# traupach/xarray_parcel

Measured on AMD Instinct MI355X. Metric: column-profiles/sec for surface_based_cape_cin, higher is better.
Workload: dtype f64

## Files before the change

xarray_parcel_amd/csrc/xp_cape_tu.hip:

```cpp
#include <hip/hip_runtime.h>

#include <cstdlib>

#include "xp_kernels.hpp"

#if !defined(XP_TU_T) || !defined(XP_TU_MODE)
#error "compile with -DXP_TU_T=<float|double> -DXP_TU_MODE=<0|1|2>"
#endif

namespace xp {
namespace {

int cape_block() {
    static int b = [] { const char *e = getenv("XP_CAPE_BLOCK"); int v = e ? atoi(e) : XP_CAPE_THREADS; return (v == 64 || v == 128 || v == 256 || v == XP_CAPE_THREADS) ? v : XP_CAPE_THREADS; }();
    return b;
}

template <typename T, int PM, int MODE, bool PERSIST> void launch_p(const CapeArgs &a, bool profile, hipStream_t s) {
    const int b = cape_block();
    unsigned nblk = (unsigned)((a.ncol + b - 1) / b);
    if (PERSIST) {
        static const int n_cu = [] { int d = 0; hipDeviceProp_t pr; return (hipGetDevice(&d) == hipSuccess && hipGetDeviceProperties(&pr, d) == hipSuccess) ? pr.multiProcessorCount : 256; }();
        unsigned cap = (unsigned)(n_cu * (b >= 1024 ? 1 : 1024 / b));
        if (nblk > cap) nblk = cap;
    }
    dim3 gr(nblk), bl(b);
    if (a.hum) {
        if (profile) hipLaunchKernelGGL((k_cape_cin<T, PM, true, MODE, true, false, false, PERSIST>), gr, bl, 0, s, a);
        else hipLaunchKernelGGL((k_cape_cin<T, PM, false, MODE, true, false, false, PERSIST>), gr, bl, 0, s, a);
        return;
    }
    if (profile) {
        if constexpr (MODE == 2) {
            const bool cc_only = !a.s.lfc_t && !a.s.el_t && !a.s.lfc_idx && !a.s.el_idx && !a.s.status;
            if (a.prof.nlev_out == 0 && a.prof.li && a.vtc && a.pos_neg && a.log_interp && cc_only) {
                hipLaunchKernelGGL((k_cape_cin<T, PM, true, MODE, false, true, true, PERSIST>), gr, bl, 0, s, a);
                return;
            }
        }
        hipLaunchKernelGGL((k_cape_cin<T, PM, true, MODE, false, false, false, PERSIST>), gr, bl, 0, s, a);
        return;
    }
    const bool lean = !a.s.lfc_t && !a.s.el_t && !a.s.lfc_idx && !a.s.el_idx && !a.s.status;
    const bool dflt = a.vtc && a.pos_neg && a.log_interp;
    if (dflt && lean) { hipLaunchKernelGGL((k_cape_cin<T, PM, false, MODE, false, true, true, PERSIST>), gr, bl, 0, s, a); return; }
    if constexpr (MODE != 2) {
        if (dflt) { hipLaunchKernelGGL((k_cape_cin<T, PM, false, MODE, false, true, false, PERSIST>), gr, bl, 0, s, a); return; }
    }
    hipLaunchKernelGGL((k_cape_cin<T, PM, false, MODE, false, false, false, PERSIST>), gr, bl, 0, s, a);
}
template <typename T, int PM, int MODE> void launch_t(const CapeArgs &a, bool profile, hipStream_t s) {
    if constexpr (MODE == 2) {
        if (a.persist) { launch_p<T, PM, MODE, true>(a, profile, s); return; }
    }
    launch_p<T, PM, MODE, false>(a, profile, s);
}

}

template <> void launch_cape_mode<XP_TU_T, XP_TU_MODE>(const CapeArgs &a, int pm, bool profile, hipStream_t s) {
    switch (pm) {
        case PM_SURFACE: launch_t<XP_TU_T, PM_SURFACE, XP_TU_MODE>(a, profile, s); break;
        case PM_MU: launch_t<XP_TU_T, PM_MU, XP_TU_MODE>(a, profile, s); break;
        case PM_ML: launch_t<XP_TU_T, PM_ML, XP_TU_MODE>(a, profile, s); break;
        default: launch_t<XP_TU_T, PM_EXPLICIT, XP_TU_MODE>(a, profile, s); break;
    }
}

}
```

xarray_parcel_amd/csrc/xp_kernels.hpp:

```cpp
#pragma once
#include "xp_level_reader.hpp"
#include "xp_profile_out.hpp"

namespace xp {

struct CapeArgs {
    View p, t, td;
    int64_t nlev, ncol;
    const void *ex_p, *ex_t, *ex_td;
    double depth;
    int vtc, log_interp, pos_neg, post_zero, table_mode;
    int hum;
    int off32;
    Tables tb;
    const double *es_tab;
    const double *fam_tab;
    int32_t *flags;
    int persist;
    int only_flagged;
    ScalarsOut s;
    ProfileOut prof;
};

enum { PM_SURFACE = 0, PM_MU = 1, PM_ML = 2, PM_EXPLICIT = 3 };


template <bool HUM> XP_DEV double as_dewpoint(const double *es, double p, double t, double m) {
    return HUM ? dewpoint_from_q_tab(es, p, t, m) : m;
}

template <typename T, bool HUM> XP_DEV Parcel select_mu_exact(const CapeArgs &a, int64_t c, const double *es, const double depth) {
    Parcel r; r.p = r.t = r.td = qnan(); r.first = a.nlev; r.idx = -1; r.prepend = false;
    double bottom = qnan(), bound = qnan(), dmin = qnan(), best = qnan();
    LookAhead<T> next(a.p, a.t, a.td, c, 0);
    for (int64_t k = 0; k < a.nlev; ++k) {
        double p, t, td;
        next.take(k + 1, a.nlev, p, t, td);
        td = as_dewpoint<HUM>(es, p, t, td);
        if (isnan_(p)) continue;
        if (isnan_(bottom)) { bottom = p; bound = bottom - depth; }
        double d = fabs(p - bound);
        bool below = p < bound;
        if (below && !(d < dmin)) break;
        if (!(d >= dmin)) dmin = d;
        double e = ln_theta_e(es, p, t, td);
        if (!isnan_(e) && !(e <= best)) { best = e; r.p = p; r.t = t; r.td = td; r.first = k; r.idx = (int)k; }
        if (below) break;
    }
    return r;
}
XP_DEV float ln_theta_e_f32(float p, float t, float td) {
    float e = 6.112f * __builtin_amdgcn_exp2f((17.67f - 4302.645f * __builtin_amdgcn_rcpf(td - 29.65f)) * 1.4426950408889634f);
    float r = 0.6219569100577033f * e * __builtin_amdgcn_rcpf(p - e);
    float l2t = __builtin_amdgcn_logf(t), l2td = __builtin_amdgcn_logf(td);
    float tl = 56.0f + __builtin_amdgcn_rcpf(__builtin_amdgcn_rcpf(td - 56.0f) + (l2t - l2td) * (0.6931471805599453f / 800.0f));
    float l2tl = __builtin_amdgcn_logf(tl);
    return 0.6931471805599453f * (l2t + (2.0f / 7.0f) * (9.965784284662087f - __builtin_amdgcn_logf(p - e)) + 0.28f * r * (l2t - l2tl)) +
// ... 85 lines not shown
    if (!closed) {
        double th_t = (pb == top) ? thb : qnan(), w_t = (pb == top) ? wb : qnan();
        layer_mean_step(s_th, pp, thp, top, th_t);
        layer_mean_step(s_w, pp, wp, top, w_t);
    }
    double dlay = fabs(top - bottom);
    double th_m = (1.0 / dlay) * s_th, w_m = (1.0 / dlay) * s_w;
    r.p = p_start;
    r.t = th_m * fpow(p_start / 1000.0, KAPPA);
    r.td = dewpoint_of_e(vapor_pressure(p_start, w_m));
    return r;
}

template <typename T, bool HUM> XP_DEV Parcel choose_parcel(const CapeArgs &a, int pmode, int64_t c, const double *es, const double depth) {
    Parcel pc;
    if (pmode == PM_SURFACE) {
        pc.p = ld<T>(a.p, 0, c); pc.t = ld<T>(a.t, 0, c); pc.td = as_dewpoint<HUM>(es, pc.p, pc.t, ld<T>(a.td, 0, c));
        pc.first = 0; pc.idx = 0; pc.prepend = false;
    } else if (pmode == PM_EXPLICIT) {
        pc.p = ld1<T>(a.ex_p, c); pc.t = ld1<T>(a.ex_t, c); pc.td = ld1<T>(a.ex_td, c);
        pc.first = 0; pc.idx = -1; pc.prepend = false;
    } else if (pmode == PM_MU) {
        pc = select_mu<T, HUM>(a, c, es, depth);
    } else {
        pc = select_ml<T, HUM>(a, c, es, depth);
    }
    return pc;
}

template <typename T, int PMODE, bool PROFILE, int MODE, bool HUM, bool DEF, bool LEAN, bool PERSIST>
__global__ __launch_bounds__(XP_CAPE_THREADS, (XP_CAPE_THREADS >= 1024 ? 4 : MODE == 2 ? 3 : PROFILE ? 4 : (PMODE == PM_SURFACE ? (HUM ? 3 : 1) : 4))) void k_cape_cin(CapeArgs a) {
    constexpr bool TABLE = (MODE == 1), FAMILY = (MODE == 2);
    constexpr bool LAZY = FAMILY && PROFILE && LEAN;
    struct Lds { double es[LDS_TAB]; double fam[FAMILY ? FAM_SIZE : 1]; double slot[SLOT_FIELDS * SLOT_STRIDE]; int next; };
    struct LdsRef { double *es, *fam, *slot; int *next; } lds;
    if constexpr (FAMILY && PROFILE) {
        __shared__ double l_es[LDS_TAB];
        __shared__ double l_fam[FAM_SIZE];
        __shared__ double l_slot[SLOT_FIELDS * SLOT_STRIDE];
        __shared__ int l_next;
        lds.es = l_es; lds.fam = l_fam; lds.slot = l_slot; lds.next = &l_next;
    } else {
        __shared__ Lds l;
        lds.es = l.es; lds.fam = l.fam; lds.slot = l.slot; lds.next = &l.next;
    }
    double *const s_es = lds.es;
    double *const s_fam = lds.fam;
    if (FAMILY) for (int i = threadIdx.x; i < FAM_SIZE; i += blockDim.x) s_fam[i] = a.fam_tab[i];
    int &s_next = *lds.next;
    if (PERSIST && threadIdx.x == 0) s_next = (int)(blockDim.x >> 6);
    int64_t c0 = (int64_t)blockIdx.x * blockDim.x + threadIdx.x;
    if (a.only_flagged) {
        int need = (c0 < a.ncol) ? a.flags[c0] : 0;
        if (!__syncthreads_or(need)) return;
        stage_es_table(a.es_tab, s_es);
        if (!need) return;
    } else {
        stage_es_table(a.es_tab, s_es);
        if (!PERSIST && c0 >= a.ncol) return;
    }
    const double *es = s_es;
    double *const s_slot = lds.slot;

    auto column = [&](const int64_t c) __attribute__((always_inline)) {
    const Parcel pc = choose_parcel<T, HUM>(a, PMODE, c, es, a.depth);

    const bool vtc = DEF || (a.vtc != 0), pos_neg = DEF || (a.pos_neg != 0), log_interp = DEF || (a.log_interp != 0);
    const bool need_w = vtc || PROFILE;
    const Lcl l = lcl(pc.p, pc.t, pc.td);
    int status = l.not_converged ? ST_LCL_NOT_CONVERGED : 0;
    const ScalarsOut &s = a.s;

    if (isnan_(l.p)) {
        if (PROFILE) ProfileSink<T, LAZY>::blank(a.prof, c);
        store_blank_column(s, c, pc, l, status);
        if (FAMILY) a.flags[c] = 0;
        return;
    }

    store_parcel_and_lcl(s, c, pc, l);
    const double vf_parcel = need_w ? virt_factor_tab(es, pc.t, pc.td, pc.p, false) : 1.0;
    const double x_lcl = log(l.p);
    const double x0 = (pc.p == l.p) ? x_lcl : log_tab<true>(es, pc.p);

    Scan sc; sc.init(l.p, x_lcl, pos_neg, s_slot + threadIdx.x);
    sc.slot[SL_LCL_T * SLOT_STRIDE] = vtc ? l.tv : l.t;
    Moist m;
    Family fam;
    if (FAMILY) fam.start(s_fam, es, l.p, x_lcl, l.t, l.tv);
    else m.start(es, l.p, x_lcl, l.t, TABLE, a.tb);
    double fam_off = l.tv - l.t;
    double fam_offp = fam_off;

    ProfileSink<T, LAZY> sink;
    constexpr bool TRACK = LEAN && PMODE == PM_ML;
    int last_k = -1, cur_k = -1;
    auto emit = [&](auto above, double P, double X, double tp, double tvp, double te, double tve, double tde, bool is_lcl) __attribute__((always_inline)) {
        if (PROFILE) sink.node(a.prof, c, es, sc, P, X, tp, tvp, te, tve, tde);
        if (TRACK) {
            if (!isnan_(P)) { last_k = (is_lcl || cur_k < 0) ? -1 : cur_k; if (is_lcl || cur_k < 0) sc.slot[SL_MIN_P * SLOT_STRIDE] = P; }
        }
        sc.template node<LEAN, decltype(above)::value>(P, X, vtc ? tvp : tp, vtc ? tve : te, is_lcl);
    };

    bool lcl_done = false;
    double *const br = sc.slot;
    clear_bracket(br);
    auto moist_node = [&](double P, double X, double T_, double m_, bool Q) __attribute__((always_inline)) {
        constexpr bool TRIO = FAMILY && LEAN && !PROFILE && !HUM && (PMODE == PM_SURFACE || PMODE == PM_EXPLICIT);
        bool f_top = false, f_any_top = false;
        const double fz = TRIO ? fam.locate(X, f_top, f_any_top) : 0.0;
        double tf = TRIO ? 0.0 : FAMILY ? fam.at(X) : m.at(P, X, a.tb, true);
        constexpr bool PARCEL_ES = TABLE;
        constexpr bool FAM_T = FAMILY && PROFILE;
        unsigned dist = table_dist(T_);
        if (!Q) dist = umax_(dist, table_dist(m_));
        if (PARCEL_ES && need_w) dist = umax_(dist, table_dist(tf));
        const bool in_range = all_in_table(dist) && (!FAM_T || LAZY || in_table(tf, 8.0));
// ... 112 lines not shown
            double Pn, Tn, Mn;
            rd.take(rem > 1, Pn, Tn, Mn);
            if (ku >= resume) {
                if (TRACK) cur_k = ku - 1;
                moist_node(sP, log_tab<true>(es, sP), sT, Q ? sM : as_dewpoint<HUM>(es, sP, sT, sM), Q);
                sP = Pn; sT = Tn; sM = Mn;
            }
        }
    } else {
        plain_walk(k);
    }
    if (TRACK) {
        if (last_k >= 0) sc.slot[SL_MIN_P * SLOT_STRIDE] = ld<T>(a.p, last_k, c);
    } else if (LEAN) {
        double pm = l.p;
        bool found = false;
        if constexpr (!SEARCH) {
            const double q = rd.peek_p();
            if (!isnan_(q)) { pm = (q < pm) ? q : pm; found = true; }
        }
        const auto late_in = late_kernargs<CapeArgs>();
        const View top_p = {late_in->p.data, late_in->p.ls, late_in->p.cs};
        for (int kk = nlev - 1; kk >= (int)pc.first; --kk) {
            if (__ballot(!found) == 0ull) break;
            const double q = ld<T>(top_p, kk, c);
            if (!found && !isnan_(q)) { pm = (q < pm) ? q : pm; found = true; }
        }
        sc.slot[SL_MIN_P * SLOT_STRIDE] = pm;
    }
    if (PROFILE) sink.finish(a.prof, c);

    const auto late = late_kernargs<CapeArgs>();
    Scan::Result r = sc.finish(late->post_zero != 0);
    if (FAMILY) late->flags[c] = fam.bad ? 1 : 0;
    store_scan_result(late->s, c, r, status | r.status);
    };

    if (PERSIST) persistent_tiles(a.ncol, s_next, column);
    else column(c0);
}

template <typename T, int PMODE> __global__ __launch_bounds__(256) void k_select_parcel(CapeArgs a) {
    __shared__ double s_es[LDS_TAB];
    const double *es = stage_es_table(a.es_tab, s_es);
    int64_t c = (int64_t)blockIdx.x * blockDim.x + threadIdx.x;
    if (c >= a.ncol) return;
    Parcel pc = choose_parcel<T, false>(a, PMODE, c, es, a.depth);
    st(a.s.par_p, a.s.f64, c, pc.p); st(a.s.par_t, a.s.f64, c, pc.t); st(a.s.par_td, a.s.f64, c, pc.td);
    sti(a.s.parcel_idx, c, pc.idx);
}

template <typename T> __global__ __launch_bounds__(256)
void k_mixed_layer(View pv, View vv, int64_t nlev, int64_t ncol, double depth_in, void *out, int f64) {
    int64_t c = (int64_t)blockIdx.x * blockDim.x + threadIdx.x;
    if (c >= ncol) return;
    double bottom = qnan(), top = qnan(), s = 0.0, pp = qnan(), vp = qnan(), pb = qnan(), vb = qnan();
    bool closed = false;
    for (int64_t k = 0; k < nlev; ++k) {
        double p = ld<T>(pv, k, c), v = ld<T>(vv, k, c);
        if (isnan_(bottom) && !isnan_(p)) { bottom = p; top = bottom - depth_in; }
        if (!isnan_(p) && p < top) {
            double cb = flog(pb), ca = flog(p), va = v;
            if (pb == top) { ca = cb; va = vb; }
            layer_mean_step(s, pp, vp, top, interp_rule(vb, va, flog(top), cb, ca));
            closed = true;
            break;
        }
        if (k > 0) layer_mean_step(s, pp, vp, p, v);
        pp = p; vp = v;
        if (!isnan_(p)) { pb = p; vb = v; }
    }
    if (!closed) layer_mean_step(s, pp, vp, top, (pb == top) ? vb : qnan());
// ... 294 lines not shown
```

xarray_parcel_amd/csrc/xp_lcl_node.hpp:

```cpp
#pragma once
#include "xp_device.hpp"

namespace xp {

struct View { const void *data; int64_t ls, cs; };
struct OutView { void *data; int64_t ls, cs; };

template <typename T> XP_DEV double ld(const View &v, int64_t k, int64_t c) {
    return (double)((const T *)v.data)[k * v.ls + c * v.cs];
}
template <typename T> XP_DEV T ldr(const View &v, int64_t k, int64_t c) { return ((const T *)v.data)[k * v.ls + c * v.cs]; }
template <typename T> XP_DEV double ld1(const void *p, int64_t c) { return (double)((const T *)p)[c]; }
XP_DEV void st(void *p, int f64, int64_t i, double v) {
    if (p == nullptr) return;
    if (f64) ((double *)p)[i] = v; else ((float *)p)[i] = (float)v;
}
XP_DEV void sti(int32_t *p, int64_t i, int v) { if (p) p[i] = v; }

struct ScalarsOut {
    void *cape, *cin, *lcl_p, *lcl_t, *lcl_tv, *lfc_p, *lfc_t, *el_p, *el_t;
    int32_t *lfc_idx, *el_idx, *status, *parcel_idx;
    void *par_p, *par_t, *par_td;
    int f64;
};
// ... 5 lines not shown
    sti(s.parcel_idx, c, pc.idx);
    st(s.par_p, s.f64, c, pc.p); st(s.par_t, s.f64, c, pc.t); st(s.par_td, s.f64, c, pc.td);
}
template <typename S> XP_DEV void store_blank_column(const S &s, int64_t c, const Parcel &pc, const Lcl &l, int status) {
    st(s.cape, s.f64, c, 0.0); st(s.cin, s.f64, c, 0.0);
    st(s.lfc_p, s.f64, c, qnan()); st(s.lfc_t, s.f64, c, qnan()); st(s.el_p, s.f64, c, qnan()); st(s.el_t, s.f64, c, qnan());
    sti(s.lfc_idx, c, -1); sti(s.el_idx, c, -1); sti(s.status, c, status);
    store_parcel_and_lcl(s, c, pc, l);
}
template <typename S> XP_DEV void store_scan_result(const S &s, int64_t c, const Scan::Result &r, int status) {
    const int f64 = s.f64;
    st(s.cape, f64, c, r.cape); st(s.cin, f64, c, r.cin);
    st(s.lfc_p, f64, c, r.lfc_p); st(s.lfc_t, f64, c, r.lfc_t);
    st(s.el_p, f64, c, r.el_p); st(s.el_t, f64, c, r.el_t);
    sti(s.lfc_idx, c, r.lfc_idx); sti(s.el_idx, c, r.el_idx); sti(s.status, c, status);
}

template <typename Args> XP_DEV const Args __attribute__((address_space(4))) *late_kernargs() {
    typedef const Args __attribute__((address_space(4))) *KernargPtr;
    KernargPtr late = (KernargPtr)__builtin_amdgcn_kernarg_segment_ptr();
    asm volatile("" : "+s"(late) : : "memory");
    return late;
}

template <typename F> XP_DEV void persistent_tiles(int64_t ncol, int &s_next, const F &column) {
    const int64_t ntiles = (ncol + 63) >> 6;
    const int t0 = (int)(ntiles * blockIdx.x / gridDim.x), t1 = (int)(ntiles * (blockIdx.x + 1) / gridDim.x);
    int tile = t0 + (int)(threadIdx.x >> 6);
    while (tile < t1) {
        const int64_t c = ((int64_t)tile << 6) + (threadIdx.x & 63);
        if (c < ncol) column(c);
        if ((threadIdx.x & 63) == 0) tile = t0 + atomicAdd(&s_next, 1);
        tile = __builtin_amdgcn_readfirstlane(tile);
    }
}

XP_DEV double interp_rule(double xb, double xa, double at, double cb, double ca) {
    double res = xb + (xa - xb) * fdiv(at - cb, ca - cb);
    return (xb == xa) ? xb : res;
}

XP_DEV void snap_to_lcl(const double *es, double lp, double x_lcl, double &P, double &X) {
    if (fabs(P - lp) <= LCL_SNAP * lp) P = lp;
    X = log_tab<true>(es, P);
    X = (P == lp) ? x_lcl : X;
}

XP_DEV void clear_bracket(double *br) {
    br[SL_BR_P * SLOT_STRIDE] = qnan(); br[SL_BR_X * SLOT_STRIDE] = qnan(); br[SL_BR_T * SLOT_STRIDE] = qnan(); br[SL_BR_TD * SLOT_STRIDE] = qnan();
}
XP_DEV void store_bracket(double *br, double P, double X, double T_, double Td_) {
    br[SL_BR_P * SLOT_STRIDE] = P; br[SL_BR_X * SLOT_STRIDE] = X; br[SL_BR_T * SLOT_STRIDE] = T_; br[SL_BR_TD * SLOT_STRIDE] = Td_;
}
XP_DEV void lcl_environment(const double *br, bool log_interp, double lp, double x_lcl, double pa, double xa, double ta, double tda,
                            double &te, double &tde) {
    const double at = log_interp ? x_lcl : lp;
    const double pb = br[SL_BR_P * SLOT_STRIDE], xb = br[SL_BR_X * SLOT_STRIDE], tb_ = br[SL_BR_T * SLOT_STRIDE], tdb = br[SL_BR_TD * SLOT_STRIDE];
    lds_wait_all();
    double cb = log_interp ? xb : pb, ca = log_interp ? xa : pa;
    if (pb == lp) { ca = cb; ta = tb_; tda = tdb; }
    te = interp_rule(tb_, ta, at, cb, ca); tde = interp_rule(tdb, tda, at, cb, ca);
}

template <bool PAIR = false> XP_DEV double virt_env_ranged(const double *es, double T_, double Td_, double P) {
    if (__builtin_amdgcn_ballot_w64(!all_in_table(umax_(table_dist(T_), table_dist(Td_)))) == 0ull) return virt_env_tab<PAIR>(es, T_, Td_, P, true);
    double tq = T_;
// ... 64 lines not shown
```

xarray_parcel_amd/csrc/xparcel.hip:

```cpp
#include <hip/hip_runtime.h>

#include <cstdarg>
#include <cstdio>
#include <cmath>
#include <cstring>
#include <cstdlib>
#include <algorithm>
#include <mutex>
#include <vector>

#include "../../include/xparcel.h"
#include "xp_kernels.hpp"
#include "xp_cape_f32.hpp"
#include "xp_multi.hpp"
#include "xp_bundle.hpp"
#include "xp_dcape.hpp"
#include "xp_kinematics.hpp"
#include "xp_effective.hpp"
#include "xp_cape_layers.hpp"
#include "xp_wind_layers.hpp"
#include "xp_thermo_layers.hpp"
#include "xp_sounding.hpp"
#include "xp_isentropic.hpp"
#include "xp_hydrostatic.hpp"
// ... 311 lines not shown
int stage_scalars(Stager &st, xp_scalars_out *s, int64_t ncol, xp::ScalarsOut *o) {
    memset(o, 0, sizeof(*o));
    if (!s) { o->f64 = 1; return 0; }
    if (s->dtype != XP_F32 && s->dtype != XP_F64) return fail(XP_E_ARG, "scalars: bad dtype");
    o->f64 = s->dtype == XP_F64;
    size_t fb = (size_t)ncol * esize(s->dtype), ib = (size_t)ncol * 4;
    int rc = 0;
#define F_(dst, src) if (!rc) rc = st.out(s->src, fb, s->mem, &o->dst)
#define I_(dst, src) if (!rc) rc = st.out(s->src, ib, s->mem, &o->dst)
    F_(cape, cape); F_(cin, cin); F_(lcl_p, lcl_pressure); F_(lcl_t, lcl_temperature); F_(lcl_tv, lcl_virtual_temperature);
    F_(lfc_p, lfc_pressure); F_(lfc_t, lfc_temperature); F_(el_p, el_pressure); F_(el_t, el_temperature);
    I_(lfc_idx, lfc_index); I_(el_idx, el_index); I_(status, status); I_(parcel_idx, parcel_index);
    F_(par_p, parcel_pressure); F_(par_t, parcel_temperature); F_(par_td, parcel_dewpoint);
#undef F_
#undef I_
    return rc;
}

struct TableSet { xp::Tables tb; const double *es, *fam; };
int snapshot_tables(bool table_mode, TableSet *t) {
    std::lock_guard<std::mutex> lk(g.mu);
    if (table_mode && !g.tables) return fail(XP_E_NO_TABLES, "Call load_moist_adiabat_lookups first.");
    *t = {g.tb, g.es_tab, g.fam_tab};
    return 0;
}

bool persist(int mode, int64_t ncol) {
    static const long long env = [] { const char *e = getenv("XP_PERSIST_MIN_COLS"); return e ? atoll(e) : -1ll; }();
    const bool searching = mode < 0 || mode == XP_PARCEL_MOST_UNSTABLE || mode == XP_PARCEL_MIXED_LAYER;
    const long long min_cols = env >= 0 ? env : searching ? (1ll << 19) : (3ll << 18);
    return (long long)ncol >= min_cols && ncol < (1ll << 36);
}

template <typename T, int PM> void launch_cape(const xp::CapeArgs &a, bool profile, hipStream_t s) {
    if (a.ncol == 0) return;
    if (a.table_mode) xp::launch_cape_mode<T, 1>(a, PM, profile, s);
    else if (a.flags) {
        xp::launch_cape_mode<T, 2>(a, PM, profile, s);
        xp::CapeArgs b = a;
        b.only_flagged = 1;
        xp::launch_cape_mode<T, 0>(b, PM, profile, s);
    } else xp::launch_cape_mode<T, 0>(a, PM, profile, s);
}
template <typename T> void launch_cape_pm(const xp::CapeArgs &a, int pm, bool profile, hipStream_t s) {
    switch (pm) {
        case XP_PARCEL_SURFACE: launch_cape<T, xp::PM_SURFACE>(a, profile, s); break;
        case XP_PARCEL_MOST_UNSTABLE: launch_cape<T, xp::PM_MU>(a, profile, s); break;
        case XP_PARCEL_MIXED_LAYER: launch_cape<T, xp::PM_ML>(a, profile, s); break;
        default: launch_cape<T, xp::PM_EXPLICIT>(a, profile, s); break;
    }
}

xp_opts default_opts() {
    xp_opts o;
    memset(&o, 0, sizeof(o));
    o.virtual_temperature_correction = 1; o.lcl_interp = XP_LCL_INTERP_LOG; o.pos_cape_neg_cin = 1; o.compute = XP_F64;
    return o;
}
int check_opts(const xp_opts &o, bool f32_ok = false) {
    if (o.lcl_interp != XP_LCL_INTERP_LINEAR && o.lcl_interp != XP_LCL_INTERP_LOG)
        return fail(XP_E_INTERP, "interpolator must be linear or log");
    if (o.moist_mode != XP_MOIST_EXACT && o.moist_mode != XP_MOIST_TABLE && o.moist_mode != XP_MOIST_FAMILY)
        return fail(XP_E_ARG, "bad moist_mode");
    if (o.compute != XP_F64 && !(f32_ok && o.compute == XP_F32))
        return fail(XP_E_ARG, o.compute == XP_F32 ? "xp_opts.compute: XP_F32 arithmetic is implemented by xp_cape_cin only" : "xp_opts.compute: XP_F32 or XP_F64");
    if (o.humidity != XP_HUM_DEWPOINT && o.humidity != XP_HUM_SPECIFIC) return fail(XP_E_ARG, "bad xp_opts.humidity");
    return 0;
}
int check_parcel(const xp_parcel *parcel) {
    if (!parcel) return fail(XP_E_ARG, "parcel: null");
    if (parcel->mode < XP_PARCEL_SURFACE || parcel->mode > XP_PARCEL_EXPLICIT) return fail(XP_E_ARG, "parcel: bad mode");
    if (parcel->mode == XP_PARCEL_EXPLICIT && (!parcel->pressure || !parcel->temperature || !parcel->dewpoint))
        return fail(XP_E_ARG, "explicit parcel: null arrays");
    return 0;
}
int check_cape(const xp_view *p, const xp_view *t, const xp_view *td, int np, const xp_parcel *parcels, const xp_opts &o, bool f32_ok = false) {
    if (int rc = check_views({{p, "pressure"}, {t, "temperature"}, {td, "dewpoint"}})) return rc;
    for (int i = 0; i < np; ++i)
        if (int rc = check_parcel(parcels + i)) return rc;
    return check_opts(o, f32_ok);
}

// ... 38 lines not shown
                const xp_opts &o, xp::CapeArgs *a, bool f32_ok = false) {
    int rc;
    if ((rc = check_cape(p, t, td, 1, parcel, o, f32_ok)) || (rc = stage_cape(st, p, t, td, o, a)) || (rc = set_parcel(st, *parcel, p, a)))
        return rc;
    return 0;
}
int stage_cape_out(Stager &st, int dtype, xp_scalars_out *scalars, xp_profile_out *profile, xp::CapeArgs *a) {
    int rc;
    if ((rc = stage_scalars(st, scalars, a->ncol, &a->s)) || !profile) return rc;
    if (profile->dtype != XP_F32 && profile->dtype != XP_F64) return fail(XP_E_ARG, "profile: bad dtype");
    if (profile->nlev_out < a->nlev + 1) return fail(XP_E_ARG, "profile: nlev_out must be >= nlev + 1");
    if (profile->mem == XP_MEM_HOST && !(profile->col_stride == 1 && profile->lev_stride == a->ncol))
        return fail(XP_E_ARG, "profile: host arrays must be dense (nlev_out, ncol)");
    void *src[6] = {profile->pressure, profile->temperature, profile->virtual_temperature,
                    profile->environment_temperature, profile->environment_virtual_temperature,
                    profile->environment_dewpoint};
    size_t b = (size_t)profile->nlev_out * (size_t)a->ncol * esize(profile->dtype);
    int rows = 0;
    for (int v = 0; v < 6; ++v) {
        if ((rc = st.out(src[v], b, profile->mem, &a->prof.v[v]))) return rc;
        rows += a->prof.v[v] != nullptr;
    }
    a->prof.nlev_out = rows ? profile->nlev_out : 0;
    a->prof.ls = profile->lev_stride; a->prof.cs = profile->col_stride;
    a->prof.f64 = profile->dtype == XP_F64;
    a->prof.native6 = rows == 6 && profile->dtype == dtype;
    if (profile->lifted_index) {
        if (!(profile->lifted_index_pressure > 0.0)) return fail(XP_E_ARG, "profile: lifted_index_pressure must be positive");
        if ((rc = st.out(profile->lifted_index, (size_t)a->ncol * esize(profile->dtype), profile->mem, &a->prof.li))) return rc;
        a->prof.li_x = log(profile->lifted_index_pressure);
    }
    return 0;
}
int family_flags(Stager &st, const xp_opts &o, int64_t ncol, int32_t **flags) {
    *flags = nullptr;
    if (o.moist_mode != XP_MOIST_FAMILY || ncol == 0) return 0;
    return st.alloc(sizeof(int32_t) * (size_t)ncol, flags);
}
void cape_pass(const Stager &st, xp::CapeArgs a, int dtype, int mode, bool profile, int32_t *flags) {
    a.flags = flags;
    a.persist = flags && persist(mode, a.ncol);
    by_dtype(dtype, [&](auto z) { launch_cape_pm<decltype(z)>(a, mode, profile, st.s); });
}

int check_compute32(const xp_view *p, const xp_parcel *parcel, const xp_opts &o, const xp_scalars_out *s, const xp_profile_out *profile) {
    if (p->dtype != XP_F32) return fail(XP_E_ARG, "xp_opts.compute = XP_F32: the views must be XP_F32");
    if (parcel->mode != XP_PARCEL_SURFACE) return fail(XP_E_ARG, "xp_opts.compute = XP_F32: parcel->mode must be XP_PARCEL_SURFACE");
    if (o.moist_mode != XP_MOIST_FAMILY) return fail(XP_E_ARG, "xp_opts.compute = XP_F32: moist_mode must be XP_MOIST_FAMILY");
    if (o.humidity != XP_HUM_DEWPOINT) return fail(XP_E_ARG, "xp_opts.compute = XP_F32: humidity must be XP_HUM_DEWPOINT");
    if (!o.virtual_temperature_correction || o.lcl_interp != XP_LCL_INTERP_LOG || !o.pos_cape_neg_cin || o.post_zero_cin)
        return fail(XP_E_ARG, "xp_opts.compute = XP_F32: virtual_temperature_correction, lcl_interp, pos_cape_neg_cin and post_zero_cin must be at their defaults");
    if (profile) return fail(XP_E_ARG, "xp_opts.compute = XP_F32: profile must be NULL");
    if (s && (s->lfc_temperature || s->el_temperature || s->lfc_index || s->el_index || s->status))
        return fail(XP_E_ARG, "xp_opts.compute = XP_F32: scalars->lfc_temperature, el_temperature, lfc_index, el_index and status must be NULL");
    return 0;
}
void cape_pass32(const Stager &st, xp::CapeArgs a, int32_t *flags) {
    if (a.ncol == 0) return;
    a.flags = flags;
    a.persist = persist(XP_PARCEL_SURFACE, a.ncol);
    xp::launch_cape_f32(a, st.s);
    a.only_flagged = 1; a.persist = 0;
    xp::launch_cape_mode<float, 0>(a, xp::PM_SURFACE, false, st.s);
}

template <typename T, int NV> void launch_interp_levels(int nt, const Stager &st, const xp::View &cv, const xp::InterpMany &m, int64_t nlev, int64_t ncol, int lg) {
    switch (nt) {
        case 1: launch(xp::k_interp_levels<T, NV, 1>, ncol, st, cv, m, nlev, ncol, lg); break;
        case 2: launch(xp::k_interp_levels<T, NV, 2>, ncol, st, cv, m, nlev, ncol, lg); break;
        case 3: launch(xp::k_interp_levels<T, NV, 3>, ncol, st, cv, m, nlev, ncol, lg); break;
        default: launch(xp::k_interp_levels<T, NV, 4>, ncol, st, cv, m, nlev, ncol, lg); break;
    }
}
template <typename T> void launch_interp_levels_v(int nv, int nt, const Stager &st, const xp::View &cv, const xp::InterpMany &m, int64_t nlev, int64_t ncol, int lg) {
    switch (nv) {
// ... 127 lines not shown
    g.tb.p_max = t->p_max; g.tb.p_step = t->p_step; g.tb.t_min = t->t_min; g.tb.t_step = t->t_step;
    g.tables = true;
    return XP_OK;
}
int xp_tables_loaded(void) { return g.tables ? 1 : 0; }

int xp_family_table(double *out, int64_t *n_lnp, int64_t *n_label) {
    DevGuard dg_;
    int rc = ensure_init();
    if (rc) return rc;
    if (n_lnp) *n_lnp = xp::FAM_COEFS / xp::FAM_NPS;
    if (n_label) *n_label = xp::FAM_NPS;
    if (out) memcpy(out, g.fam_host.data(), sizeof(double) * xp::FAM_COEFS);
    return XP_OK;
}
int xp_set_family_table(const double *tab, int64_t n_lnp, int64_t n_label) {
    DevGuard dg_;
    int rc = ensure_init();
    if (rc) return rc;
    if (!tab || n_lnp != xp::FAM_COEFS / xp::FAM_NPS || n_label != xp::FAM_NPS) return fail(XP_E_ARG, "xp_set_family_table: wrong shape");
    std::lock_guard<std::mutex> lk(g.mu);
    HIP_TRY(hipDeviceSynchronize());
    memcpy(g.fam_host.data(), tab, sizeof(double) * xp::FAM_COEFS);
    HIP_TRY(hipMemcpy(g.fam_tab, family_device_layout(g.fam_host).data(), sizeof(double) * g.fam_host.size(), hipMemcpyHostToDevice));
    return XP_OK;
}

int xp_cape_cin(const xp_view *p, const xp_view *t, const xp_view *td, const xp_parcel *parcel, const xp_opts *o,
                xp_scalars_out *scalars, xp_profile_out *profile, void *stream) {
    Entry st(stream);
    if (st.rc) return st.rc;
    const xp_opts oo = o ? *o : default_opts();
    xp::CapeArgs a;
    int32_t *flags;
    int rc;
    const bool f32 = oo.compute == XP_F32;
    if (f32 && ((rc = check_cape(p, t, td, 1, parcel, oo, true)) || (rc = check_compute32(p, parcel, oo, scalars, profile)))) return rc;
    if ((rc = fill_common(st, p, t, td, parcel, oo, &a, true)) || (rc = stage_cape_out(st, p->dtype, scalars, profile, &a)) ||
        (rc = family_flags(st, oo, a.ncol, &flags))) return rc;
    if (f32) cape_pass32(st, a, flags);
    else cape_pass(st, a, p->dtype, parcel->mode, profile != nullptr, flags);
    return st.finish();
}

int xp_cape_cin_multi(const xp_view *p, const xp_view *t, const xp_view *td, int32_t np, const xp_parcel *parcels,
                      const xp_opts *o, xp_scalars_out *scalars, xp_profile_out *profiles, void *stream) {
    Entry st(stream);
    if (st.rc) return st.rc;
    if (np < 1 || np > xp::MULTI_MAX) return fail(XP_E_ARG, "xp_cape_cin_multi: 1...%d parcels", xp::MULTI_MAX);
    if (!parcels || !scalars) return fail(XP_E_ARG, "xp_cape_cin_multi: null parcels / scalars");
    const xp_opts oo = o ? *o : default_opts();
    xp::CapeArgs a, pa[xp::MULTI_MAX];
    int rc;
    if ((rc = check_cape(p, t, td, np, parcels, oo)) || (rc = stage_cape(st, p, t, td, oo, &a))) return rc;
    for (int i = 0; i < np; ++i) {
        pa[i] = a;
        if ((rc = set_parcel(st, parcels[i], p, &pa[i])) ||
            (rc = stage_cape_out(st, p->dtype, &scalars[i], profiles ? &profiles[i] : nullptr, &pa[i]))) return rc;
    }
    const int64_t ncol = a.ncol;
    if (!multi_fused_ok(np, parcels, oo, profiles)) {
        int32_t *flags;
        if ((rc = family_flags(st, oo, ncol, &flags))) return rc;
        for (int i = 0; i < np; ++i) cape_pass(st, pa[i], p->dtype, parcels[i].mode, profiles != nullptr, flags);
        return st.finish();
    }
    xp::MultiArgs m;
    memset(&m, 0, sizeof(m));
    m.base = a;
    m.np = np;
    for (int i = 0; i < np; ++i) {
        m.mode[i] = parcels[i].mode;
        m.depth[i] = parcels[i].depth;
        m.s[i] = pa[i].s;
    }
    if (ncol == 0) return st.finish();
    int32_t *flags;
    if ((rc = st.alloc(sizeof(int32_t) * (size_t)ncol * (size_t)np, &flags))) return rc;
    for (int i = 0; i < np; ++i) m.flags[i] = flags + (size_t)i * (size_t)ncol;
    m.base.persist = persist(-1, ncol);
    by_dtype(p->dtype, [&](auto z) {
        using T = decltype(z);
        xp::launch_cape_multi<T, 2>(m, st.s);
        for (int i = 0; i < np; ++i) {
            xp::CapeArgs b = pa[i];
            b.flags = m.flags[i]; b.only_flagged = 1;
            xp::launch_cape_mode<T, 0>(b, m.mode[i], false, st.s);
        }
    });
    return st.finish();
}

int xp_conv_properties(const xp_conv_in *in, const xp_opts *o, int32_t ignore_nans, xp_conv_out *out, void *stream) {
    Entry st(stream);
    if (st.rc) return st.rc;
    if (!in || !out) return fail(XP_E_ARG, "xp_conv_properties: null argument");
// ... 20 lines not shown
        if ((rc = st.in(src[i]->data, rows_bytes(src[i], src[i]->nlev), mem, &d))) return rc;
        dv[i].data = d; dv[i].mem = XP_MEM_DEVICE;
    }
    const void *sfu, *sfv;
    if ((rc = st.in(in->surface_wind_u, cb, mem, &sfu)) || (rc = st.in(in->surface_wind_v, cb, mem, &sfv))) return rc;
    void *td, *tmp;
    int32_t *valid;
    enum { T850, T700, T500, TD850, Z700, Z500, HIU, HIV, MUP, MUTD, NTMP };
    if ((rc = st.alloc((size_t)nlev * cb, &td)) || (rc = st.alloc((size_t)NTMP * cb, &tmp)) || (rc = st.alloc((size_t)ncol * 4, &valid))) return rc;
    auto tp = [&](int i) { return (void *)((char *)tmp + (size_t)i * cb); };
    void *o_[21];
    void *const want[21] = {out->mu_cape, out->mu_cin, out->mu_mixing_ratio, out->mu_lifted_index, out->mu_dci,
                            out->mixed_100_cape, out->mixed_100_cin, out->mixed_100_lifted_index, out->mixed_100_dci,
                            out->mixed_50_cape, out->mixed_50_cin, out->mixed_50_lifted_index, out->mixed_50_dci,
                            out->lapse_rate_700_500, out->temp_500, out->freezing_level, out->melting_level,
                            out->shear_u, out->shear_v, out->shear_magnitude, (void *)out->positive_shear};
    for (int i = 0; i < 21; ++i) {
        const size_t b = i == 20 ? (size_t)ncol * 4 : cb;
        if ((rc = want[i] ? st.out(want[i], b, mem, &o_[i]) : st.alloc(b, &o_[i]))) return rc;
    }
    enum { O_MU_CAPE, O_MU_CIN, O_MU_W, O_MU_LI, O_MU_DCI, O_M1_CAPE, O_M1_CIN, O_M1_LI, O_M1_DCI, O_M5_CAPE, O_M5_CIN, O_M5_LI, O_M5_DCI,
           O_LAPSE, O_T500, O_FRZ, O_MLT, O_SHU, O_SHV, O_SHM, O_POS };
    xp::ConvColumnsArgs ca;
    memset(&ca, 0, sizeof(ca));
    ca.p = {dv[0].data, dv[0].lev_stride, dv[0].col_stride}; ca.t = {dv[1].data, dv[1].lev_stride, dv[1].col_stride};
    ca.q = {dv[2].data, dv[2].lev_stride, dv[2].col_stride}; ca.z = {dv[3].data, dv[3].lev_stride, dv[3].col_stride};
    ca.nlev = nlev; ca.ncol = ncol; ca.td = td;
    ca.t850 = tp(T850); ca.t700 = tp(T700); ca.t500 = tp(T500); ca.td850 = tp(TD850); ca.z700 = tp(Z700); ca.z500 = tp(Z500);
    ca.freezing = o_[O_FRZ]; ca.melting = o_[O_MLT]; ca.valid = valid;
    by_dtype(p->dtype, [&](auto z_) { launch(xp::k_conv_columns<decltype(z_)>, ncol, st, ca); });
    xp_view tdv = dv[0];
    tdv.data = td; tdv.lev_stride = ncol; tdv.col_stride = 1;
    xp::CapeArgs a;
    int32_t *flags;
    if ((rc = stage_cape(st, &dv[0], &dv[1], &tdv, oo, &a)) || (rc = family_flags(st, oo, ncol, &flags))) return rc;
    const struct { int mode; double depth; int cape, cin, li; } pc[3] = {{XP_PARCEL_MOST_UNSTABLE, 250.0, O_MU_CAPE, O_MU_CIN, O_MU_LI},
                                                                        {XP_PARCEL_MIXED_LAYER, 100.0, O_M1_CAPE, O_M1_CIN, O_M1_LI},
                                                                        {XP_PARCEL_MIXED_LAYER, 50.0, O_M5_CAPE, O_M5_CIN, O_M5_LI}};
    for (int i = 0; i < 3; ++i) {
        xp_scalars_out so;
        memset(&so, 0, sizeof(so));
        so.dtype = p->dtype; so.mem = XP_MEM_DEVICE; so.cape = o_[pc[i].cape]; so.cin = o_[pc[i].cin];
        if (i == 0) { so.parcel_pressure = tp(MUP); so.parcel_dewpoint = tp(MUTD); }
        xp_profile_out po;
        memset(&po, 0, sizeof(po));
        po.dtype = p->dtype; po.mem = XP_MEM_DEVICE; po.nlev_out = nlev + 1; po.lev_stride = ncol; po.col_stride = 1;
        po.lifted_index = o_[pc[i].li]; po.lifted_index_pressure = 500.0;
        xp::CapeArgs b = a;
        b.depth = pc[i].depth;
        if ((rc = stage_cape_out(st, p->dtype, &so, &po, &b))) return rc;
        cape_pass(st, b, p->dtype, pc[i].mode, true, flags);
    }
    {
        const xp_view *vars[2] = {&dv[4], &dv[5]};
        const double at6 = 6000.0;
        void *outs[2] = {tp(HIU), tp(HIV)};
        if ((rc = interp_levels(st, &dv[6], 2, vars, 1, &at6, 0, outs))) return rc;
    }
    xp::ConvFinishArgs fa;
    memset(&fa, 0, sizeof(fa));
    fa.ncol = ncol; fa.ignore_nans = ignore_nans != 0;
    fa.mu_p = tp(MUP); fa.mu_td = tp(MUTD);
    fa.li[0] = o_[O_MU_LI]; fa.li[1] = o_[O_M1_LI]; fa.li[2] = o_[O_M5_LI];
    fa.t850 = tp(T850); fa.t700 = tp(T700); fa.t500 = tp(T500); fa.td850 = tp(TD850); fa.z700 = tp(Z700); fa.z500 = tp(Z500);
    fa.hi_u = tp(HIU); fa.hi_v = tp(HIV); fa.sfc_u = sfu; fa.sfc_v = sfv; fa.valid = valid;
    fa.cape[0] = o_[O_MU_CAPE]; fa.cape[1] = o_[O_M1_CAPE]; fa.cape[2] = o_[O_M5_CAPE];
    fa.cin[0] = o_[O_MU_CIN]; fa.cin[1] = o_[O_M1_CIN]; fa.cin[2] = o_[O_M5_CIN];
    fa.li_out[0] = o_[O_MU_LI]; fa.li_out[1] = o_[O_M1_LI]; fa.li_out[2] = o_[O_M5_LI];
// ... 711 lines not shown
```

Before: 2.353 billion.

## Fuse family-mode fallback recomputation into the CAPE kernel for surface parcels

For surface and explicit parcels in family moist mode with default options and lean outputs, the kernel now recomputes flagged columns itself using the exact path. It collects per-wave ballot masks of bad columns in LDS (persistent mode) or redoes them inline, so the second only_flagged launch and the flags buffer allocation are dropped. This removes a kernel launch, a global flags round trip and the es-table restaging of the second pass. The cost is a larger fused kernel that instantiates both moist paths, which may raise register pressure and adds block-level syncs between tile batches.

```diff
diff --git a/xarray_parcel_amd/csrc/xp_cape_tu.hip b/xarray_parcel_amd/csrc/xp_cape_tu.hip
--- a/xarray_parcel_amd/csrc/xp_cape_tu.hip
+++ b/xarray_parcel_amd/csrc/xp_cape_tu.hip
@@ -41,8 +41,8 @@
         hipLaunchKernelGGL((k_cape_cin<T, PM, true, MODE, false, false, false, PERSIST>), gr, bl, 0, s, a);
         return;
     }
-    const bool lean = !a.s.lfc_t && !a.s.el_t && !a.s.lfc_idx && !a.s.el_idx && !a.s.status;
-    const bool dflt = a.vtc && a.pos_neg && a.log_interp;
+    const bool lean = cape_lean(a);
+    const bool dflt = cape_default_opts(a);
     if (dflt && lean) { hipLaunchKernelGGL((k_cape_cin<T, PM, false, MODE, false, true, true, PERSIST>), gr, bl, 0, s, a); return; }
     if constexpr (MODE != 2) {
         if (dflt) { hipLaunchKernelGGL((k_cape_cin<T, PM, false, MODE, false, true, false, PERSIST>), gr, bl, 0, s, a); return; }
diff --git a/xarray_parcel_amd/csrc/xp_kernels.hpp b/xarray_parcel_amd/csrc/xp_kernels.hpp
--- a/xarray_parcel_amd/csrc/xp_kernels.hpp
+++ b/xarray_parcel_amd/csrc/xp_kernels.hpp
@@ -23,6 +23,15 @@
 };
 
 enum { PM_SURFACE = 0, PM_MU = 1, PM_ML = 2, PM_EXPLICIT = 3 };
+
+constexpr bool family_redo_in_kernel(int mode, int pmode, bool profile, bool hum, bool deflt, bool lean) {
+    return mode == 2 && !profile && !hum && deflt && lean && (pmode == PM_SURFACE || pmode == PM_EXPLICIT);
+}
+inline bool cape_lean(const CapeArgs &a) { return !a.s.lfc_t && !a.s.el_t && !a.s.lfc_idx && !a.s.el_idx && !a.s.status; }
+inline bool cape_default_opts(const CapeArgs &a) { return a.vtc && a.pos_neg && a.log_interp; }
+inline bool family_redo_in_kernel(const CapeArgs &a, int pmode, bool profile) {
+    return family_redo_in_kernel(2, pmode, profile, a.hum != 0, cape_default_opts(a), cape_lean(a));
+}
 
 
 template <bool HUM> XP_DEV double as_dewpoint(const double *es, double p, double t, double m) {
@@ -174,17 +183,19 @@
 __global__ __launch_bounds__(XP_CAPE_THREADS, (XP_CAPE_THREADS >= 1024 ? 4 : MODE == 2 ? 3 : PROFILE ? 4 : (PMODE == PM_SURFACE ? (HUM ? 3 : 1) : 4))) void k_cape_cin(CapeArgs a) {
     constexpr bool TABLE = (MODE == 1), FAMILY = (MODE == 2);
     constexpr bool LAZY = FAMILY && PROFILE && LEAN;
-    struct Lds { double es[LDS_TAB]; double fam[FAMILY ? FAM_SIZE : 1]; double slot[SLOT_FIELDS * SLOT_STRIDE]; int next; };
-    struct LdsRef { double *es, *fam, *slot; int *next; } lds;
+    constexpr bool REDO = family_redo_in_kernel(MODE, PMODE, PROFILE, HUM, DEF, LEAN);
+    struct Lds { double es[LDS_TAB]; double fam[FAMILY ? FAM_SIZE : 1]; double slot[SLOT_FIELDS * SLOT_STRIDE]; int next;
+                 unsigned long long bad[REDO && PERSIST ? REDO_TILES : 1]; };
+    struct LdsRef { double *es, *fam, *slot; int *next; unsigned long long *bad; } lds;
     if constexpr (FAMILY && PROFILE) {
         __shared__ double l_es[LDS_TAB];
         __shared__ double l_fam[FAM_SIZE];
         __shared__ double l_slot[SLOT_FIELDS * SLOT_STRIDE];
         __shared__ int l_next;
-        lds.es = l_es; lds.fam = l_fam; lds.slot = l_slot; lds.next = &l_next;
+        lds.es = l_es; lds.fam = l_fam; lds.slot = l_slot; lds.next = &l_next; lds.bad = nullptr;
     } else {
         __shared__ Lds l;
-        lds.es = l.es; lds.fam = l.fam; lds.slot = l.slot; lds.next = &l.next;
+        lds.es = l.es; lds.fam = l.fam; lds.slot = l.slot; lds.next = &l.next; lds.bad = l.bad;
     }
     double *const s_es = lds.es;
     double *const s_fam = lds.fam;
@@ -204,7 +215,9 @@
     const double *es = s_es;
     double *const s_slot = lds.slot;
 
-    auto column = [&](const int64_t c) __attribute__((always_inline)) {
+    auto column = [&](auto mode, const CapeArgs &a, const int64_t c) __attribute__((always_inline)) -> bool {
+    constexpr bool TABLE = (decltype(mode)::value == 1), FAMILY = (decltype(mode)::value == 2);
+    constexpr bool LAZY = FAMILY && PROFILE && LEAN;
     const Parcel pc = choose_parcel<T, HUM>(a, PMODE, c, es, a.depth);
 
     const bool vtc = DEF || (a.vtc != 0), pos_neg = DEF || (a.pos_neg != 0), log_interp = DEF || (a.log_interp != 0);
@@ -216,8 +229,8 @@
     if (isnan_(l.p)) {
         if (PROFILE) ProfileSink<T, LAZY>::blank(a.prof, c);
         store_blank_column(s, c, pc, l, status);
-        if (FAMILY) a.flags[c] = 0;
-        return;
+        if (FAMILY && !REDO) a.flags[c] = 0;
+        return false;
     }
 
     store_parcel_and_lcl(s, c, pc, l);
@@ -225,7 +238,9 @@
     const double x_lcl = log(l.p);
     const double x0 = (pc.p == l.p) ? x_lcl : log_tab<true>(es, pc.p);
 
-    Scan sc; sc.init(l.p, x_lcl, pos_neg, s_slot + threadIdx.x);
+    unsigned slot_of = threadIdx.x;
+    if constexpr (REDO && PERSIST) asm volatile("" : "+v"(slot_of));
+    Scan sc; sc.init(l.p, x_lcl, pos_neg, s_slot + slot_of);
     sc.slot[SL_LCL_T * SLOT_STRIDE] = vtc ? l.tv : l.t;
     Moist m;
     Family fam;
@@ -404,12 +419,29 @@
 
     const auto late = late_kernargs<CapeArgs>();
     Scan::Result r = sc.finish(late->post_zero != 0);
-    if (FAMILY) late->flags[c] = fam.bad ? 1 : 0;
+    if (FAMILY && !REDO) late->flags[c] = fam.bad ? 1 : 0;
     store_scan_result(late->s, c, r, status | r.status);
+    return FAMILY && fam.bad;
     };
-
-    if (PERSIST) persistent_tiles(a.ncol, s_next, column);
-    else column(c0);
+    auto own = [&](const int64_t c) __attribute__((always_inline)) { return column(std::integral_constant<int, MODE>{}, a, c); };
+
+    if constexpr (REDO) {
+        auto redo = [&](int64_t c) __attribute__((always_inline)) {
+            asm volatile("" : "+v"(c));
+            column(std::integral_constant<int, 0>{}, a, c);
+        };
+        if (PERSIST) {
+            persistent_tiles_redo(a.ncol, s_next, lds.bad, own, redo);
+        } else {
+            const bool bad = own(c0);
+            if (__builtin_amdgcn_ballot_w64(bad) != 0ull) {
+                if (bad) redo((int64_t)blockIdx.x * blockDim.x + threadIdx.x);
+            }
+        }
+    } else {
+        if (PERSIST) persistent_tiles(a.ncol, s_next, own);
+        else own(c0);
+    }
 }
 
 template <typename T, int PMODE> __global__ __launch_bounds__(256) void k_select_parcel(CapeArgs a) {
diff --git a/xarray_parcel_amd/csrc/xp_lcl_node.hpp b/xarray_parcel_amd/csrc/xp_lcl_node.hpp
--- a/xarray_parcel_amd/csrc/xp_lcl_node.hpp
+++ b/xarray_parcel_amd/csrc/xp_lcl_node.hpp
@@ -61,6 +61,35 @@
         if (c < ncol) column(c);
         if ((threadIdx.x & 63) == 0) tile = t0 + atomicAdd(&s_next, 1);
         tile = __builtin_amdgcn_readfirstlane(tile);
+    }
+}
+
+constexpr int REDO_TILES = 256;
+template <typename F, typename R>
+XP_DEV void persistent_tiles_redo(int64_t ncol, int &s_next, unsigned long long *s_bad, const F &column, const R &redo) {
+    const int64_t ntiles = (ncol + 63) >> 6;
+    const int t0 = (int)(ntiles * blockIdx.x / gridDim.x), t1 = (int)(ntiles * (blockIdx.x + 1) / gridDim.x);
+    auto tid = []() __attribute__((always_inline)) { unsigned t = threadIdx.x; asm volatile("" : "+v"(t)); return t; };
+    for (int b0 = t0; b0 < t1; b0 += REDO_TILES) {
+        const int b1 = b0 + REDO_TILES < t1 ? b0 + REDO_TILES : t1;
+        int tile = b0 + (int)(threadIdx.x >> 6);
+        while (tile < b1) {
+            const int64_t c = ((int64_t)tile << 6) + (threadIdx.x & 63);
+            bool bad = false;
+            if (c < ncol) bad = column(c);
+            const unsigned long long m = __builtin_amdgcn_ballot_w64(bad);
+            if ((threadIdx.x & 63) == 0) { s_bad[tile - b0] = m; tile = b0 + atomicAdd(&s_next, 1); }
+            tile = __builtin_amdgcn_readfirstlane(tile);
+        }
+        __syncthreads();
+        if (threadIdx.x == 0) s_next = (int)(blockDim.x >> 6);
+        const int nwave = (int)(blockDim.x >> 6);
+        for (int i = b0 + __builtin_amdgcn_readfirstlane((int)(tid() >> 6)); i < b1; i += nwave) {
+            const unsigned long long m = s_bad[i - b0];
+            const unsigned lane = tid() & 63u;
+            if (m != 0ull && ((m >> lane) & 1ull)) redo(((int64_t)i << 6) + lane);
+        }
+        __syncthreads();
     }
 }
 
diff --git a/xarray_parcel_amd/csrc/xparcel.hip b/xarray_parcel_amd/csrc/xparcel.hip
--- a/xarray_parcel_amd/csrc/xparcel.hip
+++ b/xarray_parcel_amd/csrc/xparcel.hip
@@ -367,22 +367,23 @@
     return (long long)ncol >= min_cols && ncol < (1ll << 36);
 }
 
-template <typename T, int PM> void launch_cape(const xp::CapeArgs &a, bool profile, hipStream_t s) {
+template <typename T, int PM> void launch_cape(const xp::CapeArgs &a, bool profile, bool family, hipStream_t s) {
     if (a.ncol == 0) return;
     if (a.table_mode) xp::launch_cape_mode<T, 1>(a, PM, profile, s);
-    else if (a.flags) {
+    else if (family) {
         xp::launch_cape_mode<T, 2>(a, PM, profile, s);
+        if (xp::family_redo_in_kernel(a, PM, profile)) return;
         xp::CapeArgs b = a;
         b.only_flagged = 1;
         xp::launch_cape_mode<T, 0>(b, PM, profile, s);
     } else xp::launch_cape_mode<T, 0>(a, PM, profile, s);
 }
-template <typename T> void launch_cape_pm(const xp::CapeArgs &a, int pm, bool profile, hipStream_t s) {
+template <typename T> void launch_cape_pm(const xp::CapeArgs &a, int pm, bool profile, bool family, hipStream_t s) {
     switch (pm) {
-        case XP_PARCEL_SURFACE: launch_cape<T, xp::PM_SURFACE>(a, profile, s); break;
-        case XP_PARCEL_MOST_UNSTABLE: launch_cape<T, xp::PM_MU>(a, profile, s); break;
-        case XP_PARCEL_MIXED_LAYER: launch_cape<T, xp::PM_ML>(a, profile, s); break;
-        default: launch_cape<T, xp::PM_EXPLICIT>(a, profile, s); break;
+        case XP_PARCEL_SURFACE: launch_cape<T, xp::PM_SURFACE>(a, profile, family, s); break;
+        case XP_PARCEL_MOST_UNSTABLE: launch_cape<T, xp::PM_MU>(a, profile, family, s); break;
+        case XP_PARCEL_MIXED_LAYER: launch_cape<T, xp::PM_ML>(a, profile, family, s); break;
+        default: launch_cape<T, xp::PM_EXPLICIT>(a, profile, family, s); break;
     }
 }
 
@@ -487,15 +488,22 @@
     }
     return 0;
 }
-int family_flags(Stager &st, const xp_opts &o, int64_t ncol, int32_t **flags) {
-    *flags = nullptr;
+struct FamilyFlags {
+    bool family = false;
+    int32_t *redo = nullptr;
+    explicit operator bool() const { return family; }
+};
+int family_flags(Stager &st, const xp_opts &o, int64_t ncol, bool need, FamilyFlags *flags) {
+    *flags = FamilyFlags();
     if (o.moist_mode != XP_MOIST_FAMILY || ncol == 0) return 0;
-    return st.alloc(sizeof(int32_t) * (size_t)ncol, flags);
-}
-void cape_pass(const Stager &st, xp::CapeArgs a, int dtype, int mode, bool profile, int32_t *flags) {
-    a.flags = flags;
+    flags->family = true;
+    return need ? st.alloc(sizeof(int32_t) * (size_t)ncol, &flags->redo) : 0;
+}
+bool pass_needs_flags(const xp::CapeArgs &a, int mode, bool profile) { return !xp::family_redo_in_kernel(a, mode, profile); }
+void cape_pass(const Stager &st, xp::CapeArgs a, int dtype, int mode, bool profile, const FamilyFlags &flags) {
+    a.flags = flags.redo;
     a.persist = flags && persist(mode, a.ncol);
-    by_dtype(dtype, [&](auto z) { launch_cape_pm<decltype(z)>(a, mode, profile, st.s); });
+    by_dtype(dtype, [&](auto z) { launch_cape_pm<decltype(z)>(a, mode, profile, flags.family, st.s); });
 }
 
 int check_compute32(const xp_view *p, const xp_parcel *parcel, const xp_opts &o, const xp_scalars_out *s, const xp_profile_out *profile) {
@@ -689,13 +697,13 @@
     if (st.rc) return st.rc;
     const xp_opts oo = o ? *o : default_opts();
     xp::CapeArgs a;
-    int32_t *flags;
+    FamilyFlags flags;
     int rc;
     const bool f32 = oo.compute == XP_F32;
     if (f32 && ((rc = check_cape(p, t, td, 1, parcel, oo, true)) || (rc = check_compute32(p, parcel, oo, scalars, profile)))) return rc;
     if ((rc = fill_common(st, p, t, td, parcel, oo, &a, true)) || (rc = stage_cape_out(st, p->dtype, scalars, profile, &a)) ||
-        (rc = family_flags(st, oo, a.ncol, &flags))) return rc;
-    if (f32) cape_pass32(st, a, flags);
+        (rc = family_flags(st, oo, a.ncol, f32 || pass_needs_flags(a, parcel->mode, profile != nullptr), &flags))) return rc;
+    if (f32) cape_pass32(st, a, flags.redo);
     else cape_pass(st, a, p->dtype, parcel->mode, profile != nullptr, flags);
     return st.finish();
 }
@@ -717,8 +725,10 @@
     }
     const int64_t ncol = a.ncol;
     if (!multi_fused_ok(np, parcels, oo, profiles)) {
-        int32_t *flags;
-        if ((rc = family_flags(st, oo, ncol, &flags))) return rc;
+        FamilyFlags flags;
+        bool need = false;
+        for (int i = 0; i < np; ++i) need = need || pass_needs_flags(pa[i], parcels[i].mode, profiles != nullptr);
+        if ((rc = family_flags(st, oo, ncol, need, &flags))) return rc;
         for (int i = 0; i < np; ++i) cape_pass(st, pa[i], p->dtype, parcels[i].mode, profiles != nullptr, flags);
         return st.finish();
     }
@@ -805,8 +815,8 @@
     xp_view tdv = dv[0];
     tdv.data = td; tdv.lev_stride = ncol; tdv.col_stride = 1;
     xp::CapeArgs a;
-    int32_t *flags;
-    if ((rc = stage_cape(st, &dv[0], &dv[1], &tdv, oo, &a)) || (rc = family_flags(st, oo, ncol, &flags))) return rc;
+    FamilyFlags flags;
+    if ((rc = stage_cape(st, &dv[0], &dv[1], &tdv, oo, &a)) || (rc = family_flags(st, oo, ncol, true, &flags))) return rc;
     const struct { int mode; double depth; int cape, cin, li; } pc[3] = {{XP_PARCEL_MOST_UNSTABLE, 250.0, O_MU_CAPE, O_MU_CIN, O_MU_LI},
                                                                         {XP_PARCEL_MIXED_LAYER, 100.0, O_M1_CAPE, O_M1_CIN, O_M1_LI},
                                                                         {XP_PARCEL_MIXED_LAYER, 50.0, O_M5_CAPE, O_M5_CIN, O_M5_LI}};
```

After: 2.348 billion. Within noise of the previous version (-0.2%).
